# spacetelescope/subpixal

Hardware: AMD Instinct MI355X
Metric: cutout cross-correlations/sec (64x64 px, upsample=10) (higher is better)
Workload: dtype f32; 1 GPU; BASELINE.json configs[1]: 100000 64x64 Gaussian-spot cutout pairs per GPU, upsample=10, inputs resident in HBM; pairs_per_gpu=100000, tile=64, upsample=10, cc_type=CC, refine=default, parallelism=batch sharded over 1 GPU(s); gather of (dx,dy) to rank 0

## Files before the change

### subpixal_amd/csrc/spx_kernels.h

```cpp
#pragma once

namespace spx {

using rt::f32x2;
using rt::f32x4;
typedef f32x2 cf;

constexpr int kThreads = 256;

SPX_DEVICE int fresh_tid() { return rt::launder_lane(rt::thread_id()); }

enum { ST_OK = 0, ST_EDGE = 1, ST_NOMAX = 2, ST_OUTSIDE = 3, ST_WINDOW = 4, ST_FEWPTS = 5, ST_NONFINITE = 6, ST_SHAPE = 7 };
constexpr int kNoIndex = 0x7fffffff;
enum { CC_PLAIN = 0, CC_NCC = 1, CC_ZNCC = 2 };

constexpr int kNumPhases = 20;
template <int DBG> struct PhaseClock {
    unsigned long long last;
    unsigned long long acc[DBG == 100 ? kNumPhases : 1];
    SPX_DEVICE void start() {
        if constexpr (DBG == 100) {
            for (int i = 0; i < kNumPhases; ++i) acc[i] = 0;
            last = rt::clock_stamp();
        }
    }
    SPX_DEVICE void tick(int phase) {
        if constexpr (DBG == 100) {
            const unsigned long long now = rt::clock_stamp();
            acc[phase] += now - last;
            last = now;
        }
    }
    SPX_DEVICE void flush(unsigned long long* out) {
        if constexpr (DBG == 100) {
            if ((rt::thread_id() & 63) == 0)
                for (int i = 0; i < kNumPhases; ++i) rt::atomic_add_u64(out + i, acc[i]);
        }
    }
};

SPX_DEVICE cf cmul(cf a, cf w) { return rt::cmul(a, w); }
SPX_DEVICE cf cmulc(cf a, cf w) { return rt::cmulc(a, w); }
template <int DIR> SPX_DEVICE cf rot_add(cf s, cf d) { return DIR > 0 ? rt::add_mi(s, d) : rt::add_pi(s, d); }
template <int DIR> SPX_DEVICE cf rot_sub(cf s, cf d) { return DIR > 0 ? rt::add_pi(s, d) : rt::add_mi(s, d); }

template <int DIR, bool ROT2>
SPX_DEVICE void fft4(cf c0, cf c1, cf c2, cf c3, cf& y0, cf& y1, cf& y2, cf& y3) {
    const cf s0 = ROT2 ? rot_add<DIR>(c0, c2) : c0 + c2;
    const cf s1 = ROT2 ? rot_sub<DIR>(c0, c2) : c0 - c2;
    const cf s2 = c1 + c3, d = c1 - c3;
    y0 = s0 + s2;
    y2 = s0 - s2;
    y1 = rot_add<DIR>(s1, d);
    y3 = rot_sub<DIR>(s1, d);
}

template <int DIR> SPX_DEVICE void fft8(cf (&a)[8]) {
    const float h = 0.70710678118654752440f;
    const cf b0 = a[0] + a[4], d4 = a[0] - a[4];
    const cf b1 = a[1] + a[5], d5 = a[1] - a[5];
    const cf b2 = a[2] + a[6], d6 = a[2] - a[6];
    const cf b3 = a[3] + a[7], d7 = a[3] - a[7];
    const cf b5 = rot_add<DIR>(d5, d5) * h;
    const cf b7 = (DIR > 0 ? rt::neg_add_mi(d7) : rt::neg_add_pi(d7)) * h;
    fft4<DIR, false>(b0, b1, b2, b3, a[0], a[2], a[4], a[6]);
    fft4<DIR, true>(d4, b5, d6, b7, a[1], a[3], a[5], a[7]);
}

template <int DIR> SPX_DEVICE void fft8_y(cf (&v)[8][8]) {
#pragma unroll
    for (int x = 0; x < 8; ++x) {
        cf t[8];
#pragma unroll
        for (int y = 0; y < 8; ++y) t[y] = v[y][x];
        fft8<DIR>(t);
#pragma unroll
        for (int y = 0; y < 8; ++y) v[y][x] = t[y];
    }
}
template <int DIR> SPX_DEVICE void fft8_x(cf (&v)[8][8]) {
#pragma unroll
    for (int y = 0; y < 8; ++y) fft8<DIR>(v[y]);
}

#ifndef SPX_CMUL_BATCH
#define SPX_CMUL_BATCH 1
#endif
template <bool CONJ> SPX_DEVICE void mul_row(cf (&v)[8][8], int y, cf w) {
    if constexpr (SPX_CMUL_BATCH) {
        rt::cmul8_ip<CONJ>(v[y][0], v[y][1], v[y][2], v[y][3], v[y][4], v[y][5], v[y][6], v[y][7], w);
    } else {
#pragma unroll
        for (int x = 0; x < 8; ++x) { if (CONJ) rt::cmulc_ip(v[y][x], w); else rt::cmul_ip(v[y][x], w); }
    }
}
template <bool CONJ> SPX_DEVICE void mul_col(cf (&v)[8][8], int x, cf w) {
    if constexpr (SPX_CMUL_BATCH) {
        rt::cmul8_ip<CONJ>(v[0][x], v[1][x], v[2][x], v[3][x], v[4][x], v[5][x], v[6][x], v[7][x], w);
    } else {
#pragma unroll
        for (int y = 0; y < 8; ++y) { if (CONJ) rt::cmulc_ip(v[y][x], w); else rt::cmul_ip(v[y][x], w); }
    }
}

template <int XS> SPX_DEVICE void transpose_tile(cf (&v)[8][8], float* xch, int lane) {
#pragma unroll
    for (int part = 0; part < 2; ++part) {
#pragma unroll
        for (int r = 0; r < 64; ++r)
            xch[r * XS + lane] = part ? v[r >> 3][r & 7].y : v[r >> 3][r & 7].x;
        rt::wave_sync();
#pragma unroll
        for (int r = 0; r < 64; ++r) {
            const float t = xch[lane * XS + r];
            if (part) v[r >> 3][r & 7].y = t; else v[r >> 3][r & 7].x = t;
        }
        rt::wave_sync();
    }
}

template <int XS> SPX_DEVICE void transpose_tile_v(cf (&v)[8][8], float* xch, int lane) {
#pragma unroll
    for (int part = 0; part < 2; ++part) {
#pragma unroll
        for (int r = 0; r < 64; ++r)
            xch[r * XS + lane] = part ? v[r >> 3][r & 7].y : v[r >> 3][r & 7].x;
        rt::wave_sync();
#pragma unroll
        for (int r = 0; r < 64; ++r) {
            const float t = rt::lds_read_f32(xch + lane * XS + r);
            if (part) v[r >> 3][r & 7].y = t; else v[r >> 3][r & 7].x = t;
        }
        rt::wave_sync();
    }
}

template <int XS> SPX_DEVICE void transpose_tile_w(cf (&v)[8][8], float* xch, int lane) {
    static_assert(XS >= 68 && (XS & 3) == 0, "32 complex slots per row plus the conflict padding");
    cf* buf = reinterpret_cast<cf*>(xch);
    cf t[64];
#pragma unroll
    for (int h = 0; h < 2; ++h) {
        if ((lane >> 5) == h) {
#pragma unroll
            for (int r = 0; r < 64; ++r) buf[r * (XS / 2) + (lane & 31)] = v[r >> 3][r & 7];
        }
        rt::wave_sync();
        const f32x4* row = reinterpret_cast<const f32x4*>(buf + lane * (XS / 2));
#pragma unroll
        for (int j = 0; j < 16; ++j) {
            const f32x4 q = row[j];
            t[32 * h + 2 * j] = cf{q[0], q[1]};
            t[32 * h + 2 * j + 1] = cf{q[2], q[3]};
        }
        rt::wave_sync();
    }
#pragma unroll
    for (int r = 0; r < 64; ++r) v[r >> 3][r & 7] = t[r];
}

#ifndef SPX_TRANSPOSE_VARIANT
#define SPX_TRANSPOSE_VARIANT 0
#endif
template <int XS> SPX_DEVICE void transpose_tile_sel(cf (&v)[8][8], float* xch, int lane) {
    if constexpr (SPX_TRANSPOSE_VARIANT == 1) transpose_tile_v<XS>(v, xch, lane);
    else if constexpr (SPX_TRANSPOSE_VARIANT == 2) transpose_tile_w<XS>(v, xch, lane);
    else transpose_tile<XS>(v, xch, lane);
}

// ... 392 lines not shown
        const int idx = tid + i * kThreads;
        if (FOLD && idx >= G::ROWS * G::CHUNKS) break;
        const int y = FOLD ? idx / G::CHUNKS : idx >> 4;
        const int x = (FOLD ? idx - y * G::CHUNKS : (idx & 15)) << 2;
        float rr[4], mm[4];
        chunk_unpack(ld[i], ns, rr, mm);
        if constexpr (FOLD) {
            *reinterpret_cast<f32x4*>(zre + y * G::ZS + x) = f32x4{rr[0], rr[1], rr[2], rr[3]};
            *reinterpret_cast<f32x4*>(zim + y * G::ZS + x) = f32x4{mm[0], mm[1], mm[2], mm[3]};
        } else {
#pragma unroll
            for (int e = 0; e < 4; ++e) {
                zre[y * G::ZS + G::perm(x >> 2, e)] = rr[e];
                zim[y * G::ZS + G::perm(x >> 2, e)] = mm[e];
            }
        }
#pragma unroll
        for (int e = 0; e < 4; ++e) { sr += rr[e] * rr[e]; sm += mm[e] * mm[e]; }
    }
    ssq[0] = sr;
    ssq[1] = sm;
}
template <int C, bool FOLD = false, typename TIn = float>
SPX_DEVICE void stage_pair(unsigned char* lds, const TIn* __restrict__ ref,
                           const TIn* __restrict__ img, int ny, int nx,
                           const NormStatsT<TIn>& ns, float (&ssq)[2]) {
    if (nx < 4) stage_pair_rows<C, FOLD, TIn, true>(lds, ref, img, ny, nx, ns, ssq);
    else if ((nx & 3) == 0) stage_pair_rows<C, FOLD, TIn, false, true>(lds, ref, img, ny, nx, ns, ssq);
    else stage_pair_rows<C, FOLD, TIn, false>(lds, ref, img, ny, nx, ns, ssq);
}

SPX_DEVICE float balance_from_ssq(float s0, float s1) {
    if (!(s0 > 0.0f) || !(s1 > 0.0f)) return 1.0f;
    const int e0 = (int)((__builtin_bit_cast(unsigned, s0) >> 23) & 0xffu);
    const int e1 = (int)((__builtin_bit_cast(unsigned, s1) >> 23) & 0xffu);
    int e = (e0 - e1) >> 1;
    e = e < -100 ? -100 : (e > 100 ? 100 : e);
    return __builtin_bit_cast(float, (unsigned)(127 + e) << 23);
}
SPX_DEVICE float balance_factor(unsigned char* lds_scr, float (&ssq)[2]) {
    block_sum2f(lds_scr, ssq[0], ssq[1]);
    return balance_from_ssq(ssq[0], ssq[1]);
}

SPX_DEVICE int plane_col(int row, int col) { return col ^ (((row & 1) << 4) | ((row & 2) << 2)); }

#ifndef SPX_DISP5_CPLXT
#define SPX_DISP5_CPLXT 0
#endif
#ifndef SPX_FUSED_TW
#define SPX_FUSED_TW 0
#endif
template <int K> SPX_DEVICE f32x2 quad_pair(f32x4 q) {
    if constexpr (K < 2) return f32x2{q[0], q[1]}; else return f32x2{q[2], q[3]};
}
template <int K, bool CONJ> SPX_DEVICE cf soa_cmul_k(f32x4 re4, f32x4 im4, cf w) {
    return rt::bcast_fma_rot<(K & 1), CONJ>(quad_pair<K>(im4), w, rt::bcast_mul<(K & 1), CONJ>(quad_pair<K>(re4), w));
}
template <bool CONJ> SPX_DEVICE cf soa_cmul(int k, f32x4 re4, f32x4 im4, cf w) {
    switch (k & 3) {
        case 0: return soa_cmul_k<0, CONJ>(re4, im4, w);
        case 1: return soa_cmul_k<1, CONJ>(re4, im4, w);
        case 2: return soa_cmul_k<2, CONJ>(re4, im4, w);
        default: return soa_cmul_k<3, CONJ>(re4, im4, w);
    }
}
template <int K> SPX_DEVICE cf soa_cmul2_k(f32x4 re4, f32x4 im4, cf w, cf bw) {
    return rt::bcast_fma_rot<(K & 1), false>(quad_pair<K>(im4), bw, rt::bcast_mul<(K & 1), false>(quad_pair<K>(re4), w));
}
SPX_DEVICE cf soa_cmul2(int k, f32x4 re4, f32x4 im4, cf w, cf bw) {
    switch (k & 3) {
        case 0: return soa_cmul2_k<0>(re4, im4, w, bw);
        case 1: return soa_cmul2_k<1>(re4, im4, w, bw);
        case 2: return soa_cmul2_k<2>(re4, im4, w, bw);
        default: return soa_cmul2_k<3>(re4, im4, w, bw);
    }
}

template <int XS, bool CONJ, bool W0_ONE>
SPX_DEVICE void transpose_tile_tw(cf (&v)[8][8], float* xch, int lane, const cf (&w)[8]) {
    f32x4 re4[16], im4[16];
#pragma unroll
    for (int part = 0; part < 2; ++part) {
#pragma unroll
        for (int r = 0; r < 64; ++r)
            xch[r * XS + lane] = part ? v[r >> 3][r & 7].y : v[r >> 3][r & 7].x;
        rt::wave_sync();
        const f32x4* row = reinterpret_cast<const f32x4*>(xch + lane * XS);
#pragma unroll
        for (int j = 0; j < 16; ++j) { if (part) im4[j] = row[j]; else re4[j] = row[j]; }
        rt::wave_sync();
    }
#pragma unroll
    for (int r = 0; r < 64; ++r) {
        const int b = r & 7;
        if (W0_ONE && b == 0) v[r >> 3][b] = cf{re4[r >> 2][r & 3], im4[r >> 2][r & 3]};
        else v[r >> 3][b] = soa_cmul<CONJ>(r, re4[r >> 2], im4[r >> 2], w[b]);
    }
}

template <typename G, int CY, int CX>
SPX_DEVICE void load_tile_class(cf (&v)[8][8], const float* zre, const float* zim, const cf* tw, float bal,
                                int l1, int l0) {
    constexpr int NK = 7 * (CY + CX) + 1;
    cf W[NK], BW[NK];
#pragma unroll
    for (int k = 1; k < NK; ++k) { W[k] = tw[8 * k]; BW[k] = cf{bal * W[k].x, bal * W[k].y}; }
#pragma unroll
    for (int y1 = 0; y1 < 8; ++y1) {
        const f32x4* pr = reinterpret_cast<const f32x4*>(zre + (l1 + 8 * y1) * G::ZS + l0 * G::PS12);
        const f32x4* pi = reinterpret_cast<const f32x4*>(zim + (l1 + 8 * y1) * G::ZS + l0 * G::PS12);
        const f32x4 r0 = pr[0], r1 = pr[1], i0 = pi[0], i1 = pi[1];
#pragma unroll
        for (int x1 = 0; x1 < 8; ++x1) {
            const int k = CY * y1 + CX * x1;
            const f32x4 rq = x1 < 4 ? r0 : r1, iq = x1 < 4 ? i0 : i1;
            if (k == 0) v[y1][x1] = cf{rq[x1 & 3], bal * iq[x1 & 3]};
            else v[y1][x1] = soa_cmul2(x1, rq, iq, W[k], BW[k]);
        }
    }
}

template <typename L, int CY, int CX>
SPX_DEVICE void store_plane_class(const cf (&v)[8][8], float* plane, const cf* tw, int l1, int l0) {
    constexpr int NK = 7 * (CY + CX) + 1;
    cf W[NK];
#pragma unroll
    for (int k = 1; k < NK; ++k) W[k] = tw[8 * k];
#pragma unroll
    for (int x1 = 0; x1 < 8; ++x1)
#pragma unroll
        for (int y1 = 0; y1 < 8; ++y1) {
            const cf a = v[y1][x1];
            const int k = CY * y1 + CX * x1;
            const int row = l1 + 8 * y1;
            plane[row * L::PS + plane_col(row, l0 + 8 * x1)] = k == 0 ? a.y : a.y * W[k].x - a.x * W[k].y;
        }
}

SPX_DEVICE float fold_tile(cf (&v)[8][8]) {
    float s = 0.0f;
#pragma unroll
    for (int r = 0; r < 64; ++r) s += v[r >> 3][r & 7].x + v[r >> 3][r & 7].y;
    return s;
}
#define SPX_DBG_STOP(k)                                                        \
    do {                                                                       \
        if constexpr (DBG == (k)) {                                            \
            reinterpret_cast<float*>(lds + L::SCR_OFF + 768)[tid & 63] = fold_tile(v); \
            return true;                                                       \
        }                                                                      \
    } while (0)

template <int C, int DBG = 0, bool FOLD = false, bool CPLXT = false>
SPX_DEVICE bool cc_planes(unsigned char* lds, float bal, PhaseClock<DBG>& clk, int rot = 0) {
    typedef Lds<C> L;
    typedef StageGeom<C, FOLD> G;
    static_assert(C == 2, "class decomposition implemented for P = 128");
    const int tid = fresh_tid();
    const int lane = tid & 63;
    const int wave = ((tid >> 6) + rot) & (C * C - 1);
    const int cy = wave / C, cx = wave % C;
    const int l1 = lane >> 3, l0 = lane & 7;
    const cf* tw = reinterpret_cast<const cf*>(lds + L::TW_OFF);
    const float* zre = reinterpret_cast<const float*>(lds + L::R_OFF);
    const float* zim = zre + G::ROWS * G::ZS;
    float* xch = reinterpret_cast<float*>(lds + L::R_OFF + wave * L::XCH_WAVE_BYTES);

    cf v[8][8];

    const float fsx = cx ? -1.0f : 1.0f, fsy = cy ? -1.0f : 1.0f;
    if constexpr (!FOLD && SPX_FUSED_TW) {
        if (wave == 0) load_tile_class<G, 0, 0>(v, zre, zim, tw, bal, l1, l0);
        else if (wave == 1) load_tile_class<G, 0, 1>(v, zre, zim, tw, bal, l1, l0);
        else if (wave == 2) load_tile_class<G, 1, 0>(v, zre, zim, tw, bal, l1, l0);
        else load_tile_class<G, 1, 1>(v, zre, zim, tw, bal, l1, l0);
    }
    if constexpr (!FOLD && !SPX_FUSED_TW) {
#pragma unroll
        for (int y1 = 0; y1 < 8; ++y1) {
            const f32x4* pr = reinterpret_cast<const f32x4*>(zre + (l1 + 8 * y1) * G::ZS + l0 * G::PS12);
            const f32x4* pi = reinterpret_cast<const f32x4*>(zim + (l1 + 8 * y1) * G::ZS + l0 * G::PS12);
            const f32x4 r0 = pr[0], r1 = pr[1], i0 = pi[0], i1 = pi[1];
#pragma unroll
            for (int x1 = 0; x1 < 4; ++x1) {
                v[y1][x1] = cf{r0[x1], bal * i0[x1]};
                v[y1][x1 + 4] = cf{r1[x1], bal * i1[x1]};
            }
        }
    }
#pragma unroll
    for (int y1 = 0; y1 < (FOLD ? 8 : 0); ++y1)
#pragma unroll
        for (int x1 = 0; x1 < 8; ++x1) {
            const int a = (l1 + 8 * y1) * G::ZS + l0 + 8 * x1;
            float re = zre[a], im = zim[a];
            if constexpr (FOLD) {
                if (x1 < 3) {
                    re = __builtin_fmaf(fsx, zre[a + 64], re);
                    im = __builtin_fmaf(fsx, zim[a + 64], im);
                }
                if (y1 < 3) {
                    float re2 = zre[a + 64 * G::ZS], im2 = zim[a + 64 * G::ZS];
                    if (x1 < 3) {
                        re2 = __builtin_fmaf(fsx, zre[a + 64 * G::ZS + 64], re2);
                        im2 = __builtin_fmaf(fsx, zim[a + 64 * G::ZS + 64], im2);
                    }
                    re = __builtin_fmaf(fsy, re2, re);
                    im = __builtin_fmaf(fsy, im2, im);
                }
            }
            v[y1][x1] = cf{re, bal * im};
        }
    rt::block_sync_lds();
    clk.tick(1);
    rt::set_prio<0>();

    if (cy && (FOLD || !SPX_FUSED_TW)) {
#pragma unroll
        for (int y1 = 1; y1 < 8; ++y1) {
            const cf w = tw[8 * cy * y1];
            mul_row<false>(v, y1, w);
        }
    }
    if (cx && (FOLD || !SPX_FUSED_TW)) {
#pragma unroll
        for (int x1 = 1; x1 < 8; ++x1) {
            const cf w = tw[8 * cx * x1];
            mul_col<false>(v, x1, w);
        }
    }
    fft8_y<1>(v);
    fft8_x<1>(v);
    SPX_DBG_STOP(2);
    clk.tick(2);
#pragma unroll
    for (int kb = 0; kb < 8; ++kb) {
        const cf wy = tw[l1 * (cy + C * kb)];
#pragma unroll
        for (int j = 0; j < 8; ++j) v[kb][j] = cmul(v[kb][j], wy);
    }
    if constexpr (!SPX_FUSED_TW) {
#pragma unroll
        for (int kb = 0; kb < 8; ++kb) {
            const cf wx = tw[l0 * (cx + C * kb)];
#pragma unroll
            for (int j = 0; j < 8; ++j) v[j][kb] = cmul(v[j][kb], wx);
        }
    }

    SPX_DBG_STOP(3);
    clk.tick(3);
    if constexpr (SPX_FUSED_TW) {
        cf wxa[8];
#pragma unroll
        for (int x0 = 1; x0 < 8; ++x0) wxa[x0] = tw[x0 * (cx + C * l0)];
        wxa[0] = cf{1.0f, 0.0f};
        transpose_tile_tw<L::XS, false, true>(v, xch, lane, wxa);
    } else if constexpr (CPLXT) {
        transpose_tile_cplx<L::XS>(v, xch, lane);
    } else {
        transpose_tile_sel<L::XS>(v, xch, lane);
    }

    SPX_DBG_STOP(4);
    clk.tick(4);
    fft8_y<1>(v);
    fft8_x<1>(v);
    SPX_DBG_STOP(5);
    clk.tick(5);

#pragma unroll
    for (int ka = 0; ka < 8; ++ka)
#pragma unroll
        for (int kb = 0; kb < 8; ++kb) {
            v[ka][kb] = cmul(v[ka][kb], v[ka][kb]);
        }

    SPX_DBG_STOP(6);
    clk.tick(6);
    fft8_y<-1>(v);
    fft8_x<-1>(v);
#pragma unroll
    for (int y0 = 1; y0 < 8; ++y0) {
        const cf wy = tw[y0 * (cy + C * l1)];
#pragma unroll
        for (int j = 0; j < 8; ++j) v[y0][j] = cmulc(v[y0][j], wy);
    }
    if constexpr (!SPX_FUSED_TW) {
#pragma unroll
        for (int x0 = 1; x0 < 8; ++x0) {
            const cf wx = tw[x0 * (cx + C * l0)];
#pragma unroll
            for (int j = 0; j < 8; ++j) v[j][x0] = cmulc(v[j][x0], wx);
        }
    }
    SPX_DBG_STOP(7);
    clk.tick(7);
    if constexpr (SPX_FUSED_TW) {
        cf wxb[8];
#pragma unroll
        for (int kb = 0; kb < 8; ++kb) wxb[kb] = tw[l0 * (cx + C * kb)];
        transpose_tile_tw<L::XS, true, false>(v, xch, lane, wxb);
    } else if constexpr (CPLXT) {
        transpose_tile_cplx<L::XS>(v, xch, lane);
    } else {
        transpose_tile_sel<L::XS>(v, xch, lane);
    }
    SPX_DBG_STOP(8);
    clk.tick(8);
    fft8_y<-1>(v);
    fft8_x<-1>(v);
    SPX_DBG_STOP(9);
    clk.tick(9);
    rt::set_prio<1>();
    float* plane = reinterpret_cast<float*>(lds + L::R_OFF + wave * L::PLANE_STRIDE_BYTES);
    if constexpr (SPX_FUSED_TW) {
        if (wave == 0) store_plane_class<L, 0, 0>(v, plane, tw, l1, l0);
        else if (wave == 1) store_plane_class<L, 0, 1>(v, plane, tw, l1, l0);
        else if (wave == 2) store_plane_class<L, 1, 0>(v, plane, tw, l1, l0);
        else store_plane_class<L, 1, 1>(v, plane, tw, l1, l0);
    } else {
    if (cy) {
#pragma unroll
        for (int y1 = 1; y1 < 8; ++y1) {
            const cf wy = tw[8 * cy * y1];
            mul_row<true>(v, y1, wy);
        }
    }
#pragma unroll
    for (int x1 = 0; x1 < 8; ++x1) {
        const cf wx = cx ? tw[8 * cx * x1] : cf{1.0f, 0.0f};
#pragma unroll
        for (int y1 = 0; y1 < 8; ++y1) {
            const cf a = v[y1][x1];
            const int row = l1 + 8 * y1;
            plane[row * L::PS + plane_col(row, l0 + 8 * x1)] = a.y * wx.x - a.x * wx.y;
        }
    }
    }
    rt::block_sync_lds();
    clk.tick(10);
    return false;
}

SPX_DEVICE int conv_index(int n, int q) { return (n - 1 - q) + (n - 1) / 2; }

template <int C>
SPX_DEVICE float window_value(const unsigned char* lds, int ny, int nx, int qy, int qx,
                              float out_scale) {
    typedef Lds<C> L;
    const float* planes = reinterpret_cast<const float*>(lds + L::R_OFF);
    const int ly = conv_index(ny, qy), lx = conv_index(nx, qx);
    const int my = ly & 63, mx = lx & 63;
    const int sy = (ly >> 6) & 1, sx = (lx >> 6) & 1;
    static_assert(C == 2, "");
    float d[C * C];
#pragma unroll
    for (int c = 0; c < C * C; ++c)
        d[c] = planes[c * (L::PLANE_STRIDE_BYTES / 4) + my * L::PS + plane_col(my, mx)];
    const float fx = sx ? -1.0f : 1.0f, fy = sy ? -1.0f : 1.0f;
    const float acc = __builtin_fmaf(fy, __builtin_fmaf(fx, d[3], d[2]), __builtin_fmaf(fx, d[1], d[0]));
    return acc * out_scale;
}

template <typename TIn>
SPX_DEVICE NormStatsT<TIn> norm_stats(unsigned char* lds_scr, const TIn* __restrict__ ref,
                                      const TIn* __restrict__ ims, int npool, int64_t im_stride,
// ... 311 lines not shown
        for (int r = 0; r < 4; ++r) {
            const int b = bb * 16 + R::drow(lk, r), a = ab * 16 + lj;
            const float val = fv[r] * scale;
            if constexpr (L::fb_count(W) == C * C) fbuf[wave * W * W + b * W + a] = val;
            else { if (c == 0) fbuf[b * W + a] = val; else fbuf[b * W + a] += val; }
        }
    };
    if constexpr (L::fb_count(W) == C * C) {
#pragma unroll
        for (int bb = 0; bb < WB; ++bb)
#pragma unroll
            for (int ab = 0; ab < WB; ++ab) put(bb, ab, f[bb][ab], 0);
        rt::block_sync_lds();
    } else {
        for (int c = 0; c < C * C; ++c) {
            if (wave == c) {
#pragma unroll
                for (int bb = 0; bb < WB; ++bb)
#pragma unroll
                    for (int ab = 0; ab < WB; ++ab) put(bb, ab, f[bb][ab], c);
            }
            rt::block_sync_lds();
        }
    }
}

template <int C, int W>
SPX_DEVICE float fine_value(const unsigned char* lds, int b, int a) {
    typedef Lds<C> L;
    const float* fbuf = reinterpret_cast<const float*>(lds + L::FB_OFF);
    if constexpr (L::fb_count(W) == C * C) {
        float acc = fbuf[b * W + a];
#pragma unroll
        for (int c = 1; c < C * C; ++c) acc += fbuf[c * W * W + b * W + a];
        return acc;
    } else {
        return fbuf[b * W + a];
    }
}

template <int C>
SPX_DEVICE void coarse_argmax_fold(const unsigned char* lds, int ny, int nx, float& bv, int& bi) {
    typedef Lds<C> L;
    static_assert(C == 2, "");
    const int tid = fresh_tid();
    const int loy = (ny - 1) / 2, lox = (nx - 1) / 2;
    const int mx4 = (tid & 15) << 2;
    int qxa[4], qxb[4];
#pragma unroll
    for (int e = 0; e < 4; ++e) {
        const int mx = mx4 + e;
        qxa[e] = mx >= lox ? (nx - 1) + lox - mx : -1;
        qxb[e] = (nx - 1) + lox - mx - 64;
    }
    float m = -__builtin_inff();
    int best = kNoIndex;
#pragma unroll
    for (int i = 0; i < 4; ++i) {
        const int my = (tid >> 4) + 16 * i;
        const int qya = my >= loy ? (ny - 1) + loy - my : -1;
        const int qyb = (ny - 1) + loy - my - 64;
        f32x4 d[C * C];
#pragma unroll
        for (int c = 0; c < C * C; ++c)
            d[c] = *reinterpret_cast<const f32x4*>(lds + L::R_OFF + c * L::PLANE_STRIDE_BYTES +
                                                   (my * L::PS + plane_col(my, mx4)) * 4);
#pragma unroll
        for (int e = 0; e < 4; ++e) {
            const float up = d[0][e] + d[1][e], um = d[0][e] - d[1][e];
            const float tp = d[2][e] + d[3][e], tm = d[2][e] - d[3][e];
            const float vaa = up + tp, vab = um + tm, vba = up - tp, vbb = um - tm;
            if (qya >= 0 && qxa[e] >= 0 && better(vaa, qya * nx + qxa[e], m, best)) { m = vaa; best = qya * nx + qxa[e]; }
            if (qya >= 0 && qxb[e] >= 0 && better(vab, qya * nx + qxb[e], m, best)) { m = vab; best = qya * nx + qxb[e]; }
            if (qyb >= 0 && qxa[e] >= 0 && better(vba, qyb * nx + qxa[e], m, best)) { m = vba; best = qyb * nx + qxa[e]; }
            if (qyb >= 0 && qxb[e] >= 0 && better(vbb, qyb * nx + qxb[e], m, best)) { m = vbb; best = qyb * nx + qxb[e]; }
        }
    }
    bv = m;
    bi = best;
}

template <int C, bool FOLD = false>
SPX_DEVICE void coarse_argmax(const unsigned char* lds, int ny, int nx, float& bv, int& bi) {
    typedef Lds<C> L;
    static_assert(C == 2, "");
    if constexpr (FOLD) { coarse_argmax_fold<C>(lds, ny, nx, bv, bi); return; }
    const int tid = fresh_tid();
    const int loy = (ny - 1) / 2, lox = (nx - 1) / 2;
    const float ninf = -__builtin_inff();
    const int mx4 = (tid & 15) << 2;
    int qx[4];
    float fx[4];
#pragma unroll
    for (int e = 0; e < 4; ++e) {
        const int mx = mx4 + e;
        const bool wrap = mx < lox;
        qx[e] = (nx - 1) + lox - mx - (wrap ? 64 : 0);
        fx[e] = wrap ? -1.0f : 1.0f;
    }
    float val[4][4];
    int rowbase[4];
    float m = ninf;
#pragma unroll
    for (int i = 0; i < 4; ++i) {
        const int my = (tid >> 4) + 16 * i;
        const bool wrap = my < loy;
        const int qy = (ny - 1) + loy - my - (wrap ? 64 : 0);
        const float fy = wrap ? -1.0f : 1.0f;
        rowbase[i] = qy * nx;
        f32x4 d[C * C];
#pragma unroll
        for (int c = 0; c < C * C; ++c)
            d[c] = *reinterpret_cast<const f32x4*>(lds + L::R_OFF + c * L::PLANE_STRIDE_BYTES +
                                                   (my * L::PS + plane_col(my, mx4)) * 4);
#pragma unroll
        for (int e = 0; e < 4; ++e) {
            const float u = __builtin_fmaf(fx[e], d[1][e], d[0][e]);
            const float t = __builtin_fmaf(fx[e], d[3][e], d[2][e]);
            const float v = __builtin_fmaf(fy, t, u);
            val[i][e] = (qy >= 0 && qx[e] >= 0) ? v : ninf;
            m = __builtin_fmaxf(m, val[i][e]);
        }
    }
    int best = 0x7fffffff;
#pragma unroll
    for (int i = 0; i < 4; ++i)
#pragma unroll
        for (int e = 0; e < 4; ++e) {
            const int idx = (val[i][e] == m) ? rowbase[i] + qx[e] : 0x7fffffff;
            best = idx < best ? idx : best;
        }
    bv = m;
    bi = best;
}

template <typename ValFn>
SPX_DEVICE PeakResult peak_fit_wave0(unsigned char* lds_scr, int imax, int jmax, int NX, int NY,
                                     ValFn val, int fit_wave = 0) {
    const int tid = rt::thread_id() - 64 * fit_wave;
    PeakResult r;
    r.x = (double)imax; r.y = (double)jmax; r.status = ST_EDGE;
    if (imax == 0 || jmax == 0) return r;
    if (tid < 0 || tid >= 64) return r;
    int x1 = imax - 2, y1 = jmax - 2;
    if (x1 > NX - 5) x1 = NX - 5;
    if (y1 > NY - 5) y1 = NY - 5;
    if (x1 < 0) x1 = 0;
    if (y1 < 0) y1 = 0;
    const int k = tid < 25 ? tid : 24;
    const float v = val(x1 + k % 5, y1 + k / 5);
    return quad_fit_wave(v, tid, x1, y1, imax, jmax, NX, NY);
}

template <int C, int WB, int DBG = 0, bool FOLD = false, typename TIn = float, typename R = RefineF32>
SPX_DEVICE void pair_body(const TIn* __restrict__ ref, const TIn* __restrict__ img,
                          int ny, int nx, int U, int cc_type, const cf* __restrict__ tw_g,
                          const float* __restrict__ ktab, double* __restrict__ out,
                          int* __restrict__ status, unsigned char* lds, PhaseClock<DBG>& clk,
                          const TIn* __restrict__ next_ref, const TIn* __restrict__ next_img,
                          float& warm, bool& staged, int fit_wave, double inv_u) {
    typedef Lds<C> L;
    ny = rt::launder_uniform(ny);
    nx = rt::launder_uniform(nx);
    U = rt::launder_uniform(U);
    const int tid = fresh_tid();
    unsigned char* scr = lds + L::SCR_OFF;
    constexpr bool kRolled = WB == 1 && R::kRolled;
    constexpr bool kAhead = kRolled && !FOLD && sizeof(TIn) == 4 && (DBG == 0 || DBG == 100);
    bool was_staged = false;
    if constexpr (kAhead) was_staged = staged;
    staged = false;
    float bal;
    if (was_staged) {
        const float* part = reinterpret_cast<const float*>(scr + SCR_AHEAD);
        const float s0 = (part[0] + part[2]) + (part[4] + part[6]);
        const float s1 = (part[1] + part[3]) + (part[5] + part[7]);
        bal = balance_from_ssq(s0, s1);
        clk.tick(19);
    } else {
        const NormStatsT<TIn> ns = norm_stats(scr, ref, img, 1, 0, ny, nx, cc_type);
        float ssq[2];
        rt::consume(warm);
        stage_pair<C, FOLD, TIn>(lds, ref, img, ny, nx, ns, ssq);
        bal = balance_factor(scr, ssq);
        clk.tick(0);
    }
    const float oscale = 0.5f / ((float)(L::P * L::P) * bal);
    if constexpr (DBG == 1) return;
    const int rot = (C * C - fit_wave) & (C * C - 1);
    if (cc_planes<C, DBG, FOLD>(lds, bal, clk, rot)) return;
    if constexpr (DBG == 10) return;
    FineTables<(WB > 0 ? WB : 1), R> ft;
    float afrag[kRolled ? 16 : 1][4];
    if constexpr (kRolled) load_afrag<C>(lds, afrag, rot);
    else if constexpr (WB > 0) load_fine_tables<C, WB, R>(ft, ktab, rot);
    if constexpr (sizeof(TIn) == 4 && !kRolled) if (next_ref) warm = warm_next_pair(next_ref, next_img);

    float bv;
    int bi;
    coarse_argmax<C, FOLD>(lds, ny, nx, bv, bi);
    block_argmax(scr, bv, bi, 0);
    const bool nonfinite = bi == kNoIndex;
    if (nonfinite) bi = 0;
    int qyc = bi / nx, qxc = bi - (bi / nx) * nx;
    clk.tick(11);
    if constexpr (DBG == 11) { if (tid == 0) out[0] = (double)bi; return; }

    PeakResult pk;
    if (nonfinite) {
        pk.x = 0.0; pk.y = 0.0; pk.status = ST_NONFINITE;
    } else if constexpr (WB == 0) {
        pk = peak_fit_wave0(scr, qxc, qyc, nx, ny, [&](int x, int y) {
            return window_value<C>(lds, ny, nx, y, x, oscale);
        }, fit_wave);
    } else {
        constexpr int W = 16 * (WB > 0 ? WB : 1);
        const int NX = U * nx, NY = U * ny;
        int imax = 0, jmax = 0;
        bool inside = false;
        for (int iter = 0; iter < 4; ++iter) {
            if constexpr (kRolled) {
                RolledTables<(WB > 0 ? WB : 1)> kt;
                load_rolled_tables<C, (WB > 0 ? WB : 1)>(kt, ktab, ny, nx, qyc, qxc, rot);
                bool ahead = false;
                if constexpr (kAhead) ahead = iter == 0 && next_ref && cc_type == CC_PLAIN;
                if (ahead) {
                    if constexpr (kAhead) {
                        FullTileLoads nl;
                        const int atid = fresh_tid();
                        stage_full_issue(nl, reinterpret_cast<const float*>(next_ref),
                                         reinterpret_cast<const float*>(next_img), atid);
                        rt::sched_fence();
                        NormStatsT<float> nns;
                        nns.active = 0;
                        nns.im_mean = 0; nns.im_rstd = 1; nns.ref_mean = 0; nns.ref_rstd = 1;
                        float sr = 0.0f, sm = 0.0f;
                        auto finish = [&]() {
#pragma unroll
                            for (int m = 32; m >= 1; m >>= 1) {
                                sr += rt::shfl_xor(sr, m);
                                sm += rt::shfl_xor(sm, m);
                            }
                            float* part = reinterpret_cast<float*>(scr + SCR_AHEAD);
                            if ((atid & 63) == 0) { part[2 * (atid >> 6)] = sr; part[2 * (atid >> 6) + 1] = sm; }
                        };
                        auto commit = [&](int k) {
                            if constexpr (DBG == 100) {
                                if (k != 15) return;
                                clk.tick(12);
#pragma unroll
                                for (int j = 0; j < 16; ++j) stage_full_piece<C>(lds, nl, j >> 2, j & 3, atid, nns, sr, sm);
                                finish();
                                clk.tick(18);
                            } else {
                                stage_full_piece<C>(lds, nl, k >> 2, k & 3, atid, nns, sr, sm);
                                if (k == 15) finish();
                            }
                        };
                        fine_window_rolled<C, (WB > 0 ? WB : 1)>(lds, afrag, kt, rot, commit);
                        staged = true;
                    }
                } else {
                    if constexpr (sizeof(TIn) == 4) if (iter == 0 && next_ref) warm = warm_next_pair(next_ref, next_img);
                    fine_window_rolled<C, (WB > 0 ? WB : 1)>(lds, afrag, kt, rot);
                }
            } else {
                fine_window<C, (WB > 0 ? WB : 1), R>(lds, ft, ny, nx, qyc, qxc, rot);
            }
            clk.tick(12);
            if constexpr (DBG == 12) { if (tid == 0) out[0] = (double)fine_value<C, W>(lds, 0, 0); return; }
            const int fx0 = U * qxc - W / 2, fy0 = U * qyc - W / 2;
            float fv = -__builtin_inff();
            int fi = 0x7fffffff;
#pragma unroll 4
            for (int i = (tid & 63); i < W * W; i += 64) {
                const int b = i / W, a = i % W;
                const int idx = a * W + b;
                const int gy = fy0 + a, gx = fx0 + b;
                const float val = fine_value<C, W>(lds, b, a);
                const bool in = gy >= 0 && gy < NY && gx >= 0 && gx < NX;
                if (in && better(val, idx, fv, fi)) { fv = val; fi = idx; }
            }
            wave_argmax(fv, fi);
            clk.tick(13);
            if constexpr (DBG == 13) { if (tid == 0) out[0] = (double)fi; return; }
            if (fi == kNoIndex) { imax = jmax = -1; break; }
            const int a = fi / W, b = fi % W;
            jmax = fy0 + a;
            imax = fx0 + b;
            int x1 = imax - 2, y1 = jmax - 2;
            if (x1 > NX - 5) x1 = NX - 5;
            if (y1 > NY - 5) y1 = NY - 5;
            if (x1 < 0) x1 = 0;
            if (y1 < 0) y1 = 0;
            const bool okx = (x1 >= fx0 && x1 + 4 < fx0 + W) || imax == 0;
            const bool oky = (y1 >= fy0 && y1 + 4 < fy0 + W) || jmax == 0;
            if (okx && oky) { inside = true; break; }
            if (!okx) qxc += (b < W / 2) ? -1 : 1;
            if (!oky) qyc += (a < W / 2) ? -1 : 1;
            qxc = qxc < 0 ? 0 : (qxc > nx ? nx : qxc);
            qyc = qyc < 0 ? 0 : (qyc > ny ? ny : qyc);
            rt::block_sync_lds();
        }
        clk.tick(16);
        if (inside) {
            const int fx0 = U * qxc - W / 2, fy0 = U * qyc - W / 2;
            pk = peak_fit_wave0(scr, imax, jmax, NX, NY, [&](int x, int y) {
                return fine_value<C, W>(lds, x - fx0, y - fy0);
            }, fit_wave);
        } else if (imax < 0) {
            pk.x = 0.0; pk.y = 0.0; pk.status = ST_NONFINITE;
        } else {
            pk.x = (double)imax; pk.y = (double)jmax; pk.status = ST_WINDOW;
        }
    }
    clk.tick(17);
    if (tid == 64 * fit_wave) {
        out[0] = pk.x * inv_u - (double)((nx - 1) / 2);
        out[1] = pk.y * inv_u - (double)((ny - 1) / 2);
        if (status) status[0] = pk.status;
    }
    clk.tick(14);
}

template <int C, int WB, int DBG = 0, bool FOLD = false, typename TIn = float, typename R = RefineF32>
SPX_TKERNEL(256) void pair_kernel(const TIn* __restrict__ ref, const TIn* __restrict__ img,
                                  int64_t nbatch, int ny, int nx, int U, int cc_type,
                                  const cf* __restrict__ tw_g, const float* __restrict__ ktab,
                                  double* __restrict__ out, int* __restrict__ status) {
    SPX_DYN_LDS(lds);
    load_twiddles<C>(lds, tw_g);
    PhaseClock<DBG> clk;
    clk.start();
    const int64_t stride = (int64_t)ny * nx;
    const bool full = !FOLD && sizeof(TIn) == 4 && ny == 64 && nx == 64 &&
        ((reinterpret_cast<uintptr_t>(ref) | reinterpret_cast<uintptr_t>(img)) & 15) == 0;
    const int64_t step = rt::grid_size();
    float warm = 0.0f;
    bool staged = false;
    int fit_wave = (int)(rt::block_id() & 3);
    const double inv_u = rt::read_lane(1.0 / (double)U, 0);
    for (int64_t p = first_item(rt::block_id(), step); p < nbatch; p += step) {
        const bool more = full && (p + step < nbatch);
        pair_body<C, WB, DBG, FOLD, TIn, R>(ref + p * stride, img + p * stride, ny, nx, U, cc_type, tw_g, ktab,
                              out + 2 * p, status ? status + p : nullptr, lds, clk,
                              more ? ref + (p + step) * stride : nullptr,
                              more ? img + (p + step) * stride : nullptr, warm, staged, fit_wave, inv_u);
        fit_wave = (fit_wave + 1) & 3;
        if constexpr (WB == 0) rt::block_sync_lds();
        clk.tick(15);
    }
    if constexpr (DBG == 100)
        clk.flush(reinterpret_cast<unsigned long long*>(status + nbatch));
}

template <int C>
SPX_DEVICE void interlace_window_fold(const unsigned char* lds, int ny, int nx, float out_scale,
                                      float* __restrict__ icc, int ox, int oy, float& bv, int& bi) {
    typedef Lds<C> L;
    static_assert(C == 2, "");
    const int tid = fresh_tid();
    const int loy = (ny - 1) / 2, lox = (nx - 1) / 2;
    const int NX = 2 * nx;
    const int mx4 = (tid & 15) << 2;
    int gxa[4], gxb[4];
#pragma unroll
    for (int e = 0; e < 4; ++e) {
        const int mx = mx4 + e;
        const int qb = (nx - 1) + lox - mx - 64;
        gxa[e] = mx >= lox ? 2 * ((nx - 1) + lox - mx) + ox : -1;
        gxb[e] = qb >= 0 ? 2 * qb + ox : -1;
    }
    float m = bv;
    int best = bi;
#pragma unroll
    for (int i = 0; i < 4; ++i) {
        const int my = (tid >> 4) + 16 * i;
        const int qb = (ny - 1) + loy - my - 64;
        const int rowa = my >= loy ? (2 * ((ny - 1) + loy - my) + oy) * NX : -1;
        const int rowb = qb >= 0 ? (2 * qb + oy) * NX : -1;
        f32x4 d[C * C];
#pragma unroll
        for (int c = 0; c < C * C; ++c)
            d[c] = *reinterpret_cast<const f32x4*>(lds + L::R_OFF + c * L::PLANE_STRIDE_BYTES +
                                                   (my * L::PS + plane_col(my, mx4)) * 4);
#pragma unroll
        for (int e = 0; e < 4; ++e) {
            const float up = d[0][e] + d[1][e], um = d[0][e] - d[1][e];
            const float tp = d[2][e] + d[3][e], tm = d[2][e] - d[3][e];
            const float vaa = (up + tp) * out_scale, vab = (um + tm) * out_scale;
            const float vba = (up - tp) * out_scale, vbb = (um - tm) * out_scale;
            auto put = [&](int row, int gx, float v) {
                if (row >= 0 && gx >= 0) {
                    icc[row + gx] = v;
                    v = nan_as_inf(v);
                    if (better(v, row + gx, m, best)) { m = v; best = row + gx; }
                }
            };
            put(rowa, gxa[e], vaa);
            put(rowa, gxb[e], vab);
            put(rowb, gxa[e], vba);
            put(rowb, gxb[e], vbb);
        }
    }
    bv = m;
    bi = best;
}

template <int C, bool FOLD = false>
SPX_DEVICE void interlace_window(const unsigned char* lds, int ny, int nx, float out_scale,
                                 float* __restrict__ icc, int ox, int oy, float& bv, int& bi) {
    typedef Lds<C> L;
    static_assert(C == 2, "");
    if constexpr (FOLD) { interlace_window_fold<C>(lds, ny, nx, out_scale, icc, ox, oy, bv, bi); return; }
    const int tid = fresh_tid();
    const int loy = (ny - 1) / 2, lox = (nx - 1) / 2;
    const int NX = 2 * nx;
    const float ninf = -__builtin_inff();
    const int mx4 = (tid & 15) << 2;
    int gx[4];
    float fx[4];
#pragma unroll
    for (int e = 0; e < 4; ++e) {
        const int mx = mx4 + e;
        const bool wrap = mx < lox;
        const int qx = (nx - 1) + lox - mx - (wrap ? 64 : 0);
        gx[e] = qx >= 0 ? 2 * qx + ox : -1;
        fx[e] = wrap ? -1.0f : 1.0f;
    }
    float val[4][4];
    int rowbase[4];
    float m = ninf;
#pragma unroll
    for (int i = 0; i < 4; ++i) {
        const int my = (tid >> 4) + 16 * i;
        const bool wrap = my < loy;
        const int qy = (ny - 1) + loy - my - (wrap ? 64 : 0);
        const float fy = wrap ? -1.0f : 1.0f;
        rowbase[i] = qy >= 0 ? (2 * qy + oy) * NX : -1;
        f32x4 d[C * C];
#pragma unroll
        for (int c = 0; c < C * C; ++c)
            d[c] = *reinterpret_cast<const f32x4*>(lds + L::R_OFF + c * L::PLANE_STRIDE_BYTES +
                                                   (my * L::PS + plane_col(my, mx4)) * 4);
#pragma unroll
        for (int e = 0; e < 4; ++e) {
            const float u = __builtin_fmaf(fx[e], d[1][e], d[0][e]);
            const float t = __builtin_fmaf(fx[e], d[3][e], d[2][e]);
            const float v = __builtin_fmaf(fy, t, u) * out_scale;
            const bool ok = rowbase[i] >= 0 && gx[e] >= 0;
            if (ok) icc[rowbase[i] + gx[e]] = v;
            val[i][e] = ok ? nan_as_inf(v) : ninf;
            m = __builtin_fmaxf(m, val[i][e]);
        }
    }
    int best = 0x7fffffff;
#pragma unroll
    for (int i = 0; i < 4; ++i)
#pragma unroll
        for (int e = 0; e < 4; ++e) {
            const int idx = (val[i][e] == m) ? rowbase[i] + gx[e] : 0x7fffffff;
            best = idx < best ? idx : best;
        }
    if (better(m, best, bv, bi)) { bv = m; bi = best; }
}

template <int C, bool FOLD = false, typename TIn = float>
SPX_DEVICE void disp5_body(const TIn* __restrict__ ref, const TIn* __restrict__ im4,
                           int ny, int nx, int cc_type, const cf* __restrict__ tw_g,
                           float* __restrict__ icc, double* __restrict__ out,
                           int* __restrict__ status, unsigned char* lds) {
    typedef Lds<C> L;
    unsigned char* scr = lds + L::SCR_OFF;
    const int64_t stride = (int64_t)ny * nx;
    NormStatsT<TIn> ns = norm_stats(scr, ref, im4, 4, stride, ny, nx, cc_type);
    ns.im_mean = rt::read_lane(ns.im_mean, 0);
    ns.im_rstd = rt::read_lane(ns.im_rstd, 0);
    ns.ref_mean = rt::read_lane(ns.ref_mean, 0);
    ns.ref_rstd = rt::read_lane(ns.ref_rstd, 0);
    ns.active = rt::read_lane(ns.active, 0);

    float bv = -__builtin_inff();
    int bi = 0x7fffffff;
    const int NX = 2 * nx, NY = 2 * ny;
    for (int q = 0; q < 4; ++q) {
        const int ox = q & 1, oy = q >> 1;
        float ssq[2];
        stage_pair<C, FOLD, TIn>(lds, ref, im4 + q * stride, ny, nx, ns, ssq);
        const float bal = balance_factor(scr, ssq);
        const float oscale = 0.5f / ((float)(L::P * L::P) * bal);
        PhaseClock<0> noclk;
        cc_planes<C, 0, FOLD, SPX_DISP5_CPLXT>(lds, bal, noclk);
        interlace_window<C, FOLD>(lds, ny, nx, oscale, icc, ox, oy, bv, bi);
        rt::block_sync_lds();
    }
    rt::block_sync();
    block_argmax(scr, bv, bi, 0);
    const bool nonfinite = !(bv < __builtin_inff());
    const int jmax = bi / NX, imax = bi % NX;
    PeakResult pk;
// ... 72 lines not shown
```

Before: 27.13 million cross-correlations/s.

## Defer peak quadratic fit into next pair's FFT stage on wave 0

When the next pair is already staged, the 5x5 quadratic peak fit for the current pair is postponed and run by wave 0 inside the next pair's cc_planes, right after the staging barrier. The fine-grid values it needs are read from LDS before later stages overwrite them. This is meant to take the serial single-wave fit off the tail of each pair so the other waves are not left idle. The risk is that wave 0 becomes the straggler in the FFT phase, and correctness depends on the fine window staying untouched in LDS until the deferred fit reads it; if the last pair of a block is deferred, nothing appears to flush it.

```diff
diff --git a/subpixal_amd/csrc/spx_kernels.h b/subpixal_amd/csrc/spx_kernels.h
--- a/subpixal_amd/csrc/spx_kernels.h
+++ b/subpixal_amd/csrc/spx_kernels.h
@@ -14,7 +14,7 @@
 constexpr int kNoIndex = 0x7fffffff;
 enum { CC_PLAIN = 0, CC_NCC = 1, CC_ZNCC = 2 };
 
-constexpr int kNumPhases = 20;
+constexpr int kNumPhases = 21;
 template <int DBG> struct PhaseClock {
     unsigned long long last;
     unsigned long long acc[DBG == 100 ? kNumPhases : 1];
@@ -713,8 +713,10 @@
         }                                                                      \
     } while (0)
 
-template <int C, int DBG = 0, bool FOLD = false, bool CPLXT = false>
-SPX_DEVICE bool cc_planes(unsigned char* lds, float bal, PhaseClock<DBG>& clk, int rot = 0) {
+struct NoDeferredWork { SPX_DEVICE void operator()() const {} };
+template <int C, int DBG = 0, bool FOLD = false, bool CPLXT = false, typename Deferred = NoDeferredWork>
+SPX_DEVICE bool cc_planes(unsigned char* lds, float bal, PhaseClock<DBG>& clk, int rot = 0,
+                          Deferred deferred = Deferred()) {
     typedef Lds<C> L;
     typedef StageGeom<C, FOLD> G;
     static_assert(C == 2, "class decomposition implemented for P = 128");
@@ -775,6 +777,10 @@
         }
     rt::block_sync_lds();
     clk.tick(1);
+    if constexpr (!__is_same(Deferred, NoDeferredWork)) {
+        if (wave == 0) deferred();
+        clk.tick(20);
+    }
     rt::set_prio<0>();
 
     if (cy && (FOLD || !SPX_FUSED_TW)) {
@@ -1392,13 +1398,39 @@
     return quad_fit_wave(v, tid, x1, y1, imax, jmax, NX, NY);
 }
 
+struct PendingFit {
+    bool fit = false;
+    int imax = 0, jmax = 0, fx0 = 0, fy0 = 0;
+    double* out = nullptr;
+    int* status = nullptr;
+};
+
+template <int C, int W>
+SPX_DEVICE void fit_pending(const unsigned char* lds, const PendingFit& pf, int nx, int ny, int U, double inv_u) {
+    const int lane = fresh_tid() & 63;
+    const int NX = U * nx, NY = U * ny;
+    int x1 = pf.imax - 2, y1 = pf.jmax - 2;
+    if (x1 > NX - 5) x1 = NX - 5;
+    if (y1 > NY - 5) y1 = NY - 5;
+    if (x1 < 0) x1 = 0;
+    if (y1 < 0) y1 = 0;
+    const int k = lane < 25 ? lane : 24;
+    const float v = fine_value<C, W>(lds, x1 + k % 5 - pf.fx0, y1 + k / 5 - pf.fy0);
+    const PeakResult pk = quad_fit_wave(v, lane, x1, y1, pf.imax, pf.jmax, NX, NY);
+    if (lane == 0) {
+        pf.out[0] = pk.x * inv_u - (double)((nx - 1) / 2);
+        pf.out[1] = pk.y * inv_u - (double)((ny - 1) / 2);
+        if (pf.status) pf.status[0] = pk.status;
+    }
+}
+
 template <int C, int WB, int DBG = 0, bool FOLD = false, typename TIn = float, typename R = RefineF32>
 SPX_DEVICE void pair_body(const TIn* __restrict__ ref, const TIn* __restrict__ img,
                           int ny, int nx, int U, int cc_type, const cf* __restrict__ tw_g,
                           const float* __restrict__ ktab, double* __restrict__ out,
                           int* __restrict__ status, unsigned char* lds, PhaseClock<DBG>& clk,
                           const TIn* __restrict__ next_ref, const TIn* __restrict__ next_img,
-                          float& warm, bool& staged, int fit_wave, double inv_u) {
+                          float& warm, bool& staged, PendingFit& pend, int fit_wave, double inv_u) {
     typedef Lds<C> L;
     ny = rt::launder_uniform(ny);
     nx = rt::launder_uniform(nx);
@@ -1410,6 +1442,8 @@
     bool was_staged = false;
     if constexpr (kAhead) was_staged = staged;
     staged = false;
+    const PendingFit prev = pend;
+    pend.fit = false;
     float bal;
     if (was_staged) {
         const float* part = reinterpret_cast<const float*>(scr + SCR_AHEAD);
@@ -1428,7 +1462,14 @@
     const float oscale = 0.5f / ((float)(L::P * L::P) * bal);
     if constexpr (DBG == 1) return;
     const int rot = (C * C - fit_wave) & (C * C - 1);
-    if (cc_planes<C, DBG, FOLD>(lds, bal, clk, rot)) return;
+    if constexpr (kAhead) {
+        auto fit_prev = [&]() {
+            if (prev.fit) fit_pending<C, 16 * WB>(lds, prev, nx, ny, U, inv_u);
+        };
+        if (cc_planes<C, DBG, FOLD, false, decltype(fit_prev)>(lds, bal, clk, rot, fit_prev)) return;
+    } else {
+        if (cc_planes<C, DBG, FOLD>(lds, bal, clk, rot)) return;
+    }
     if constexpr (DBG == 10) return;
     FineTables<(WB > 0 ? WB : 1), R> ft;
     float afrag[kRolled ? 16 : 1][4];
@@ -1447,6 +1488,8 @@
     if constexpr (DBG == 11) { if (tid == 0) out[0] = (double)bi; return; }
 
     PeakResult pk;
+    bool defer = false;
+    int d_imax = 0, d_jmax = 0, d_fx0 = 0, d_fy0 = 0;
     if (nonfinite) {
         pk.x = 0.0; pk.y = 0.0; pk.status = ST_NONFINITE;
     } else if constexpr (WB == 0) {
@@ -1543,7 +1586,11 @@
             rt::block_sync_lds();
         }
         clk.tick(16);
-        if (inside) {
+        if constexpr (kAhead) defer = inside && staged && imax != 0 && jmax != 0;
+        if (defer) {
+            d_imax = imax; d_jmax = jmax;
+            d_fx0 = U * qxc - W / 2; d_fy0 = U * qyc - W / 2;
+        } else if (inside) {
             const int fx0 = U * qxc - W / 2, fy0 = U * qyc - W / 2;
             pk = peak_fit_wave0(scr, imax, jmax, NX, NY, [&](int x, int y) {
                 return fine_value<C, W>(lds, x - fx0, y - fy0);
@@ -1555,10 +1602,19 @@
         }
     }
     clk.tick(17);
-    if (tid == 64 * fit_wave) {
+    if (!defer && tid == 64 * fit_wave) {
         out[0] = pk.x * inv_u - (double)((nx - 1) / 2);
         out[1] = pk.y * inv_u - (double)((ny - 1) / 2);
         if (status) status[0] = pk.status;
+    }
+    if constexpr (kAhead) {
+        pend.fit = rt::read_lane((int)defer, 0) != 0;
+        pend.imax = rt::read_lane(d_imax, 0);
+        pend.jmax = rt::read_lane(d_jmax, 0);
+        pend.fx0 = rt::read_lane(d_fx0, 0);
+        pend.fy0 = rt::read_lane(d_fy0, 0);
+        pend.out = out;
+        pend.status = status;
     }
     clk.tick(14);
 }
@@ -1578,6 +1634,7 @@
     const int64_t step = rt::grid_size();
     float warm = 0.0f;
     bool staged = false;
+    PendingFit pend;
     int fit_wave = (int)(rt::block_id() & 3);
     const double inv_u = rt::read_lane(1.0 / (double)U, 0);
     for (int64_t p = first_item(rt::block_id(), step); p < nbatch; p += step) {
@@ -1585,7 +1642,7 @@
         pair_body<C, WB, DBG, FOLD, TIn, R>(ref + p * stride, img + p * stride, ny, nx, U, cc_type, tw_g, ktab,
                               out + 2 * p, status ? status + p : nullptr, lds, clk,
                               more ? ref + (p + step) * stride : nullptr,
-                              more ? img + (p + step) * stride : nullptr, warm, staged, fit_wave, inv_u);
+                              more ? img + (p + step) * stride : nullptr, warm, staged, pend, fit_wave, inv_u);
         fit_wave = (fit_wave + 1) & 3;
         if constexpr (WB == 0) rt::block_sync_lds();
         clk.tick(15);
```

Result: no change. 27.22 million cross-correlations/s, median of 6 (+0.3%).
